# cambridge-mlg/RECOMBINER

Measured on AMD Instinct MI355X. Metric: INRs trained/sec (whole node) + PSNR@bpp vs reference, CIFAR-10, higher is better.
Workload: dtype bf16; 1 GPU; CIFAR-10 32x32, 4096 INRs/GPU, 3x32 SIREN (in 32 = 16 Fourier + 16 upsampled pe), S=1, training_mappings=True, Adam lr 2e-4; inrs_per_gpu=4096, parallelism=datapoint-sharded x1, tuned_library_gemms=True

## Files before the change

### recombiner_amd/csrc/upconv.hip

```cpp
#include "rcb_common.h"

using namespace rcb;

typedef float f32x16 __attribute__((ext_vector_type(16)));
typedef __bf16 bf16x8 __attribute__((ext_vector_type(8)));
typedef __bf16 bf16x4 __attribute__((ext_vector_type(4)));
typedef short s16x4 __attribute__((ext_vector_type(4)));

namespace {

constexpr int CIN = 64;
#ifndef RCB_UP_HOT
#define RCB_UP_HOT 0
#endif
#ifndef RCB_UP_NOSTORE
#define RCB_UP_NOSTORE 0
#endif
#ifndef RCB_B3_PF
#define RCB_B3_PF 2
#endif
#ifndef RCB_UP_PF
#define RCB_UP_PF 3
#endif
constexpr int XRS = 72;
// ... 588 lines not shown
  }
  if (b < a.batch) {
    RCB_STAGED2(img)
    if (b + gs < a.batch) RCB_FETCHD2(b + gs)
  }
  __syncthreads();
  int cur = 0;
  for (; b < a.batch; b += gs, cur ^= 1) {
    const __bf16* im = img + cur * (IMGB / 2);
    D2_T(0);
    if (b + gs < a.batch) {
      __bf16* nx = img + (cur ^ 1) * (IMGB / 2);
      RCB_STAGED2(nx)
      if (b + 2 * gs < a.batch) RCB_FETCHD2(b + 2 * gs)
    }
    D2_T(1);
    const long long xoff = ((long long)b * G * G + pos) * CIN + 32 * mt + 16 * h;
    float xf[16];
    Frag xb[2];
    if (kh == 0) {
      if (X_F32) {
#pragma unroll
        for (int k = 0; k < 4; ++k) {
          const float4 t = reinterpret_cast<const float4*>(reinterpret_cast<const float*>(a.x) + xoff)[k];
          xf[4 * k] = t.x; xf[4 * k + 1] = t.y; xf[4 * k + 2] = t.z; xf[4 * k + 3] = t.w;
        }
      } else {
        xb[0].u = reinterpret_cast<const uint4*>(reinterpret_cast<const __bf16*>(a.x) + xoff)[0];
        xb[1].u = reinterpret_cast<const uint4*>(reinterpret_cast<const __bf16*>(a.x) + xoff)[1];
      }
    }
    f32x16 acc;
#pragma unroll
    for (int r = 0; r < 16; ++r) acc[r] = 0.f;
#pragma unroll
    for (int c = 0; c < 8; ++c) {
      const int n = 8 * kh + c, ry = (n >> 2) - 1, rx = (n & 3) - 1;
      const int xx = 2 * v + rx + 1, sw = (xx >> 1) & 7;
      const __bf16* px = im + (2 * u + ry + 1) * ROWS + xx * RS;
      uint4 curf[4];
#pragma unroll
      for (int kb = 0; kb < 4; ++kb) curf[kb] = *reinterpret_cast<const uint4*>(px + 8 * ((2 * kb + h) ^ sw));
#pragma unroll
      for (int kb = 0; kb < 4; ++kb) {
        Frag bf, fa;
        bf.u = curf[kb];
        fa.u = fr[c][kb];
        acc = mfma16(fa.v, bf.v, acc);
      }
      __builtin_amdgcn_sched_barrier(0);
    }
    D2_T(3);
    float* rw = red + (cur * 4 + (wave & 3)) * 16 * 64;
    if (kh == 1) {
#pragma unroll
      for (int r = 0; r < 16; ++r) rw[r * 64 + lane] = acc[r];
    }
    D2_T(4);
    __syncthreads();
    D2_T(5);
    if (kh == 0) {
#pragma unroll
      for (int r = 0; r < 16; ++r) acc[r] += rw[r * 64 + lane];
#pragma unroll
      for (int hf = 0; hf < 2; ++hf) {
        float o[8];
#pragma unroll
        for (int k = 0; k < 4; ++k) {
          auto sw = __builtin_amdgcn_permlane32_swap(__float_as_uint(acc[4 * hf + k]), __float_as_uint(acc[8 + 4 * hf + k]),
                                                     false, false);
          o[k] = __uint_as_float(sw[0]);
          o[4 + k] = __uint_as_float(sw[1]);
        }
        if (X_F32) {
#pragma unroll
          for (int k = 0; k < 8; ++k) {
            o[k] *= (xf[8 * hf + k] > 0.f ? 1.0f : SLOPE);
            dbsum[8 * hf + k] += o[k];
          }
          float4* dst = reinterpret_cast<float4*>(reinterpret_cast<float*>(a.dx) + xoff + 8 * hf);
          dst[0] = make_float4(o[0], o[1], o[2], o[3]);
          dst[1] = make_float4(o[4], o[5], o[6], o[7]);
        } else {
          Frag oo;
#pragma unroll
          for (int k = 0; k < 8; ++k) {
            oo.v[k] = (__bf16)(o[k] * ((float)xb[hf].v[k] > 0.f ? 1.0f : SLOPE));
            dbsum[8 * hf + k] += (float)oo.v[k];
          }
          if (RCB_UP_NOSTORE != 2 || a.batch < 0) reinterpret_cast<uint4*>(reinterpret_cast<__bf16*>(a.dx) + xoff)[hf] = oo.u;
        }
      }
    }
    D2_T(6);
  }
#if RCB_D2_STAMPS
  ph_[7] = __builtin_amdgcn_s_memrealtime() - t_loop_;
  ph_[2] = t_loop_ - t_entry_;
  if (blockIdx.x == 0 && lane == 0)
    for (int k = 0; k < 8; ++k) g_d2_stamps[wave * 8 + k] = ph_[k];
#endif
#undef RCB_FETCHD2
#undef RCB_STAGED2
  if (dbias_partial) {
    __syncthreads();
#pragma unroll
    for (int k = 0; k < 16; ++k) {
#pragma unroll
      for (int off = 16; off > 0; off >>= 1) dbsum[k] += __shfl_xor(dbsum[k], off, 64);
    }
    float* r2 = red;
    if (kh == 0 && q == 0) {
#pragma unroll
      for (int k = 0; k < 16; ++k) r2[tile * 64 + 32 * mt + 16 * h + k] = dbsum[k];
    }
    __syncthreads();
    if (tid < 64) dbias_partial[(long long)blockIdx.x * 64 + tid] = r2[tid] + r2[64 + tid];
  }
}

struct WgradArgs {
  const void* x;
  const void* dy;
  float* partial;
  int batch;
};

__device__ __forceinline__ s16x4 tr_read(const __bf16* p) {
  return __builtin_amdgcn_ds_read_tr16_b64_v4i16((__attribute__((address_space(3))) s16x4*)p);
}

template <int COUT>
__device__ __forceinline__ void bias_partials_join(const float (&dbsum)[8], float* red, int tid, float* dst) {
  constexpr int C8 = COUT / 8, NG = 512 / COUT;
  __syncthreads();
#pragma unroll
  for (int j = 0; j < 8; ++j) red[tid * 8 + j] = dbsum[j];
  __syncthreads();
  {
    const int ch = tid % COUT, grp = tid / COUT;
    const int c8 = ch >> 3, j = ch & 7;
    float sacc = 0.f;
#pragma unroll
    for (int k = 0; k < 8; ++k) sacc += red[(c8 + C8 * (8 * grp + k)) * 8 + j];
    red[512 * 8 + grp * COUT + ch] = sacc;
  }
  __syncthreads();
  if (tid < COUT) {
    float tot = 0.f;
#pragma unroll
    for (int g = 0; g < NG; ++g) tot += red[512 * 8 + g * COUT + tid];
    dst[tid] = tot;
  }
}

template <int COUT, int G, int X_MODE, int DY_F32>
__global__ void __launch_bounds__(512) upconv_wgrad_kernel(WgradArgs a) {
  constexpr int NT = (COUT + 31) / 32;
  WC_T(0, 0);
  constexpr int HG = G + 2;
  constexpr int OG = 2 * G;
  constexpr int DM = DY_F32 ? 2 : 0;
  constexpr int NX = G * G * (CIN / 8) / 512, ND = OG * OG * (COUT / 8) / 512;
  static_assert(NX * 512 == G * G * (CIN / 8) && ND * 512 == OG * OG * (COUT / 8) && 512 % (COUT / 8) == 0, "tiling");
  constexpr int WSZ = 1024 * COUT, ROW = WSZ + COUT;
  extern __shared__ __attribute__((aligned(16))) unsigned char smem_raw[];
  __bf16* ximg = reinterpret_cast<__bf16*>(smem_raw);
  constexpr int DRS = COUT == 64 ? XRS : COUT;
  __bf16* dimg = ximg + HG * HG * XRS;
  const int tid = threadIdx.x, wave = tid >> 6, lane = tid & 63;
  const int h = lane >> 5, fb = (lane >> 4) & 1, i16 = lane & 15, q4 = i16 >> 2, p4 = i16 & 3;
  for (int e = tid; e < HG * HG * XRS / 8; e += 512) reinterpret_cast<uint4*>(ximg)[e] = make_uint4(0, 0, 0, 0);
  f32x16 acc[2][2][NT];
#pragma unroll
  for (int c = 0; c < 2; ++c)
#pragma unroll
    for (int mt = 0; mt < 2; ++mt)
#pragma unroll
      for (int nt = 0; nt < NT; ++nt)
#pragma unroll
        for (int r = 0; r < 16; ++r) acc[c][mt][nt][r] = 0.f;
  float dbsum[8];
#pragma unroll
  for (int j = 0; j < 8; ++j) dbsum[j] = 0.f;
  Raw8<X_MODE> px[NX];
  Raw8<DM> pd[ND];
#define RCB_WG_FETCH(bb)                                                                                   \
  {                                                                                                        \
    _Pragma("unroll") for (int k = 0; k < NX; ++k)                                                         \
        px[k] = raw_load<X_MODE>(a.x, (long long)(bb) * G * G * CIN + 8 * (tid + 512 * k));                \
    _Pragma("unroll") for (int k = 0; k < ND; ++k)                                                         \
        pd[k] = raw_load<DM>(a.dy, (long long)(bb) * OG * OG * COUT + 8 * (tid + 512 * k));                \
  }
  int b = blockIdx.x;
  if (b < a.batch) RCB_WG_FETCH(b)
  WC_T(0, 1);
  for (; b < a.batch; b += gridDim.x) {
    __syncthreads();
#pragma unroll
    for (int k = 0; k < NX; ++k) {
      const int e = tid + 512 * k, pix = e >> 3, c8 = e & 7;
      const int i = pix / G, j = pix - i * G;
      Frag f;
      f.v = raw_frag<X_MODE>(px[k], true);
      *reinterpret_cast<uint4*>(ximg + ((i + 1) * HG + (j + 1)) * XRS + 8 * c8) = f.u;
    }
#pragma unroll
    for (int k = 0; k < ND; ++k) {
      Frag f;
      f.v = raw_frag<DM>(pd[k], true);
      const int e = tid + 512 * k;
      *reinterpret_cast<uint4*>(dimg + (e / (COUT / 8)) * DRS + 8 * (e % (COUT / 8))) = f.u;
#pragma unroll
      for (int j = 0; j < 8; ++j) dbsum[j] += (float)f.v[j];
    }
    __syncthreads();
    if (b + (int)gridDim.x < a.batch) RCB_WG_FETCH(b + gridDim.x)
    {
      const int p = wave >> 1, pa = p >> 1, pb = p & 1, ty = wave & 1;
      for (int pt = 0; pt < G * G / 32; ++pt) {
#pragma unroll
        for (int ks = 0; ks < 2; ++ks) {
          union { s16x4 s[2]; bf16x8 v; } av[2][2], bv[NT];
#pragma unroll
          for (int w2 = 0; w2 < 2; ++w2) {
            const int pos = 32 * pt + 16 * ks + 8 * h + 4 * w2 + q4;
            const int i = pos / G, j = pos - i * G;
            const __bf16* xr = ximg + ((i + pa + ty) * HG + (j + pb)) * XRS + 16 * fb + 4 * p4;
#pragma unroll
            for (int c = 0; c < 2; ++c)
#pragma unroll
              for (int mt = 0; mt < 2; ++mt) av[c][mt].s[w2] = tr_read(xr + c * XRS + 32 * mt);
            const __bf16* dr = dimg + ((2 * i + pa) * OG + (2 * j + pb)) * DRS + 4 * p4;
#pragma unroll
            for (int nt = 0; nt < NT; ++nt) bv[nt].s[w2] = tr_read(dr + ((COUT >= 32) ? (32 * nt + 16 * fb) : 0));
          }
#pragma unroll
          for (int c = 0; c < 2; ++c)
#pragma unroll
            for (int mt = 0; mt < 2; ++mt)
#pragma unroll
              for (int nt = 0; nt < NT; ++nt) acc[c][mt][nt] = mfma16(av[c][mt].v, bv[nt].v, acc[c][mt][nt]);
        }
      }
    }
  }
#undef RCB_WG_FETCH
  WC_T(0, 2);
  float* slab = a.partial + (long long)blockIdx.x * ROW;
  bias_partials_join<COUT>(dbsum, reinterpret_cast<float*>(smem_raw), tid, slab + WSZ);
#pragma unroll
  for (int c = 0; c < 2; ++c) {
    const int combo = 2 * wave + c;
    const int p = combo >> 2, t = combo & 3;
#pragma unroll
    for (int mt = 0; mt < 2; ++mt)
#pragma unroll
      for (int nt = 0; nt < NT; ++nt) {
        const int co = 32 * nt + (lane & 31);
        if (co < COUT) {
#pragma unroll
          for (int r = 0; r < 16; ++r) {
            const int ci = 32 * mt + rho(r, h);
            slab[weff_index(t >> 1, t & 1, ci, p >> 1, p & 1, co, COUT)] = acc[c][mt][nt][r];
          }
        }
      }
  }
  WC_T(0, 3);
}

#ifndef RCB_B3_STAMPS
#define RCB_B3_STAMPS 0
#endif
#ifndef RCB_B3_WG16
#define RCB_B3_WG16 1
#endif
#ifndef RCB_B3_DIAG
#define RCB_B3_DIAG 0
#endif
#if RCB_B3_STAMPS
__device__ unsigned long long g_b3_stamps[8 * 8];
#define B3_T(k)                                                     \
  do {                                                              \
    const unsigned long long now_ = __builtin_amdgcn_s_memtime();   \
    ph_[k] += now_ - last_;                                         \
    last_ = now_;                                                   \
  } while (0)
#else
#define B3_T(k) do { } while (0)
#endif

struct Bwd3Args {
  const void* dy;
  const float* weff;
  const void* x;
  void* dx;
  float* partial;
  int batch;
  const uint4* pack;
};

__global__ void __launch_bounds__(512) upconv_bwd3_fused_kernel(Bwd3Args a) {
  constexpr int COUT = 16, G = 16, OG = 32, HO = 34, RS = 24, HG = 18, NF = 32;
#if RCB_B3_STAMPS
  const unsigned long long t_entry_ = __builtin_amdgcn_s_memrealtime();
#endif
  constexpr int WSZ = 1024 * COUT, ROW = WSZ + COUT;
#if RCB_B3_WG16
  constexpr int XR3 = 64;
#define B3_XKEY(col) ((((col) >> 1) & 1) | ((((col) >> 3) & 1) << 1))
#else
  constexpr int XR3 = XRS;
#define B3_XKEY(col) 0
#endif
  extern __shared__ __attribute__((aligned(16))) unsigned char smem_raw[];
  uint4* frags = reinterpret_cast<uint4*>(smem_raw);
  __bf16* dyimg = reinterpret_cast<__bf16*>(smem_raw + NF * 1024);
  __bf16* ximg = dyimg + HO * HO * RS;
  constexpr int SCR_RS = 40;
  __bf16* dxscr = ximg + HG * HG * XR3;
  const int tid = threadIdx.x, wave = tid >> 6, lane = tid & 63, q = lane & 31, h = lane >> 5;
  const int fb = (lane >> 4) & 1, i16 = lane & 15, q4 = i16 >> 2, p4 = i16 & 3;
  if (a.pack) {
    uint4 t4[NF * 64 / 512];
#pragma unroll
    for (int k = 0; k < NF * 64 / 512; ++k) t4[k] = a.pack[20480 + tid + 512 * k];
#pragma unroll
    for (int k = 0; k < NF * 64 / 512; ++k) frags[tid + 512 * k] = t4[k];
  }
  for (int e = tid; e < (a.pack ? 0 : NF * 64); e += 512) {
    const int ln = e & 63, slot = e >> 6;
    const int mt = slot & 1, combo = slot >> 1;
    const int ry = (combo >> 2) - 1, rx = (combo & 3) - 1;
    const int pa = (ry & 1), ty = (ry <= 0) ? 1 : 0;
    const int pb = (rx & 1), tx = (rx <= 0) ? 1 : 0;
    const int fq = ln & 31, fh = ln >> 5, ci = 32 * mt + fq;
    Frag f;
#pragma unroll
    for (int j = 0; j < 8; ++j) f.v[j] = (__bf16)a.weff[weff_index(ty, tx, ci, pa, pb, 8 * fh + j, COUT)];
    frags[e] = f.u;
  }
  for (int e = tid; e < (HO * HO * RS + HG * HG * XR3) / 8; e += 512) reinterpret_cast<uint4*>(dyimg)[e] = make_uint4(0, 0, 0, 0);
#if RCB_B3_WG16
  f32x4v wacc[2][4];
#pragma unroll
  for (int c = 0; c < 2; ++c)
#pragma unroll
    for (int cb = 0; cb < 4; ++cb)
#pragma unroll
      for (int r = 0; r < 4; ++r) wacc[c][cb][r] = 0.f;
#else
  f32x16 wacc[2][2];
#pragma unroll
  for (int c = 0; c < 2; ++c)
#pragma unroll
    for (int mt = 0; mt < 2; ++mt)
#pragma unroll
      for (int r = 0; r < 16; ++r) wacc[c][mt][r] = 0.f;
#endif
  float dbsum[8];
#pragma unroll
  for (int j = 0; j < 8; ++j) dbsum[j] = 0.f;
  uint4 pdy[4], px[4];
#pragma unroll
  for (int k = 0; k < 4; ++k) pdy[k] = px[k] = make_uint4(0, 0, 0, 0);
#define RCB_FETCH_B3(bb)                                                                                               \
  {                                                                                                                   \
    const uint4* sd_ = reinterpret_cast<const uint4*>(reinterpret_cast<const __bf16*>(a.dy) + (long long)(bb) * OG * OG * COUT); \
    const uint4* sx_ = reinterpret_cast<const uint4*>(reinterpret_cast<const __bf16*>(a.x) + (long long)(bb) * G * G * CIN);    \
    _Pragma("unroll") for (int k = 0; k < 4; ++k) { pdy[k] = sd_[tid + 512 * k]; px[k] = sx_[tid + 512 * k]; }         \
  }
  const int gs = gridDim.x;
  int b = blockIdx.x;
  __syncthreads();
  if (b < a.batch) RCB_FETCH_B3(b)
  const int u = (wave * 32 + q) >> 4, v = (wave * 32 + q) & 15;
#if RCB_B3_STAMPS
  unsigned long long ph_[8] = {0, 0, 0, 0, 0, 0, 0, 0}, last_ = __builtin_amdgcn_s_memtime();
  ph_[5] = __builtin_amdgcn_s_memrealtime();
#endif
  for (; b < a.batch; b += gs) {
    __syncthreads();
    B3_T(0);
#pragma unroll
    for (int k = 0; k < 4; ++k) {
      const int e = tid + 512 * k;
      {
        const int pix = e >> 1, c8 = e & 1;
        *reinterpret_cast<uint4*>(dyimg + (((pix >> 5) + 1) * HO + ((pix & 31) + 1)) * RS + 8 * c8) = pdy[k];
        Frag f;
        f.u = pdy[k];
#pragma unroll
        for (int j = 0; j < 8; ++j) dbsum[j] += (float)f.v[j];
      }
      {
        const int pix = e >> 3, c8 = e & 7;
        *reinterpret_cast<uint4*>(ximg + (((pix >> 4) + 1) * HG + ((pix & 15) + 1)) * XR3 + 16 * ((c8 >> 1) ^ B3_XKEY((pix & 15) + 1)) + 8 * (c8 & 1)) = px[k];
      }
    }
    B3_T(1);
    __syncthreads();
    B3_T(2);
    if (b + gs < a.batch) RCB_FETCH_B3(b + gs)
    {
      f32x16 acc[2];
#pragma unroll
      for (int mt = 0; mt < 2; ++mt)
#pragma unroll
        for (int r = 0; r < 16; ++r) acc[mt][r] = 0.f;
      constexpr int B3_PF = RCB_B3_PF;
      uint4 rg[B3_PF + 1][3];
      auto tap_reads = [&](int n, uint4 (&dst)[3]) {
        const int ry = (n >> 2) - 1, rx = (n & 3) - 1;
        dst[0] = *reinterpret_cast<const uint4*>(dyimg + ((2 * u + ((RCB_B3_DIAG == 3) ? 0 : ry) + 1) * HO + (2 * v + ((RCB_B3_DIAG == 3) ? 0 : rx) + 1)) * RS + 8 * h);
        dst[1] = frags[((RCB_B3_DIAG == 2 ? 0 : n) * 2 + 0) * 64 + lane];
        dst[2] = frags[((RCB_B3_DIAG == 2 ? 0 : n) * 2 + 1) * 64 + lane];
      };
#pragma unroll
      for (int n = 0; n < B3_PF; ++n) tap_reads(n, rg[n]);
#pragma unroll
      for (int n = 0; n < 16; ++n) {
        if (n + B3_PF < 16) tap_reads(n + B3_PF, rg[(n + B3_PF) % (B3_PF + 1)]);
        __builtin_amdgcn_sched_barrier(0);
        Frag bf, fa;
        bf.u = rg[n % (B3_PF + 1)][0];
#pragma unroll
        for (int mt = 0; mt < 2; ++mt) {
          fa.u = rg[n % (B3_PF + 1)][1 + mt];
          acc[mt] = mfma16(fa.v, bf.v, acc[mt]);
        }
        __builtin_amdgcn_sched_barrier(0);
      }
      const __bf16* xs = ximg + ((u + 1) * HG + (v + 1)) * XR3;
      const int xk16 = 16 * B3_XKEY(v + 1);
      __bf16* scr = dxscr + wave * (32 * SCR_RS);
      __bf16* dxw = reinterpret_cast<__bf16*>(a.dx) + ((long long)(RCB_B3_DIAG == 4 ? (int)blockIdx.x : b) * G * G + wave * 32) * CIN;
#pragma unroll
      for (int mt = 0; mt < 2; ++mt) {
#pragma unroll
        for (int g4 = 0; g4 < 4; ++g4) {
          const int ci = 32 * mt + 8 * g4 + 4 * h;
          const bf16x4 t = *reinterpret_cast<const bf16x4*>(xs + (((32 * mt + 8 * g4) & ~15) ^ xk16) + ((8 * g4) & 15) + 4 * h);
          bf16x4 ob;
#pragma unroll
          for (int k = 0; k < 4; ++k) ob[k] = (__bf16)(acc[mt][4 * g4 + k] * ((float)t[k] > 0.f ? 1.0f : SLOPE));
          *reinterpret_cast<bf16x4*>(scr + q * SCR_RS + 8 * g4 + 4 * h) = ob;
        }
        __builtin_amdgcn_fence(__ATOMIC_ACQ_REL, "wavefront");
#pragma unroll
        for (int ps = 0; ps < 2; ++ps) {
          const int pl = 16 * ps + (lane >> 2), ch = lane & 3;
          const uint4 o = *reinterpret_cast<const uint4*>(scr + pl * SCR_RS + 8 * ch);
          if (RCB_B3_DIAG != 1 || a.batch < 0) *reinterpret_cast<uint4*>(dxw + pl * CIN + 32 * mt + 8 * ch) = o;
        }
        __builtin_amdgcn_fence(__ATOMIC_ACQ_REL, "wavefront");
      }
    }
    __builtin_amdgcn_sched_barrier(0);
    B3_T(3);
#if RCB_B3_WG16
    {
      const int p = wave >> 1, pa = p >> 1, pb = p & 1, ty = wave & 1, kg = lane >> 4;
      typedef __attribute__((address_space(3))) s16x4* lds_tr_t;
      unsigned xa[2][2][4], da[2];
#pragma unroll
      for (int w2 = 0; w2 < 2; ++w2) {
        const int pos = 8 * kg + 4 * w2 + q4;
        const int i = pos >> 4, j = pos & 15;
#pragma unroll
        for (int c = 0; c < 2; ++c) {
          const int col = j + pb + c;
#pragma unroll
          for (int cb = 0; cb < 4; ++cb) {
            xa[w2][c][cb] = (unsigned)(size_t)(lds_tr_t)(ximg + ((i + pa + ty) * HG + col) * XR3 + 16 * (cb ^ B3_XKEY(col)) + 4 * p4);
            asm volatile("" : "+v"(xa[w2][c][cb]));
          }
        }
        da[w2] = (unsigned)(size_t)(lds_tr_t)(dyimg + ((2 * i + pa + 1) * HO + (2 * j + pb + 1)) * RS + 4 * p4);
        asm volatile("" : "+v"(da[w2]));
      }
      constexpr unsigned XSTEP = 2 * HG * XR3 * 2, DSTEP = 4 * HO * RS * 2;
#pragma unroll 1
      for (int trip = 0; trip < G * G / 64; ++trip) {
#pragma unroll
        for (int u2 = 0; u2 < 2; ++u2) {
          union { s16x4 s[2]; bf16x8 v; } av[2][4], bv;
#pragma unroll
          for (int w2 = 0; w2 < 2; ++w2) {
#pragma unroll
            for (int c = 0; c < 2; ++c)
#pragma unroll
              for (int cb = 0; cb < 4; ++cb)
                av[c][cb].s[w2] = __builtin_amdgcn_ds_read_tr16_b64_v4i16((lds_tr_t)(size_t)(xa[w2][c][cb] + (2 * trip + u2) * XSTEP));
            bv.s[w2] = __builtin_amdgcn_ds_read_tr16_b64_v4i16((lds_tr_t)(size_t)(da[w2] + (2 * trip + u2) * DSTEP));
          }
#pragma unroll
          for (int c = 0; c < 2; ++c)
#pragma unroll
            for (int cb = 0; cb < 4; ++cb) wacc[c][cb] = mfma16x32(av[c][cb].v, bv.v, wacc[c][cb]);
        }
      }
    }
#else
    {
      const int p = wave >> 1, pa = p >> 1, pb = p & 1, ty = wave & 1;
#pragma unroll 2
      for (int pt = 0; pt < G * G / 32; ++pt) {
#pragma unroll
        for (int ks = 0; ks < 2; ++ks) {
          union { s16x4 s[2]; bf16x8 v; } av[2][2], bv;
#pragma unroll
          for (int w2 = 0; w2 < 2; ++w2) {
            const int pos = 32 * pt + 16 * ks + 8 * h + 4 * w2 + q4;
            const int i = pos >> 4, j = pos & 15;
            const __bf16* xr = ximg + ((i + pa + ty) * HG + (j + pb)) * XRS + 16 * fb + 4 * p4;
#pragma unroll
            for (int c = 0; c < 2; ++c)
#pragma unroll
              for (int mt = 0; mt < 2; ++mt) av[c][mt].s[w2] = tr_read(xr + c * XRS + 32 * mt);
            bv.s[w2] = tr_read(dyimg + ((2 * i + pa + 1) * HO + (2 * j + pb + 1)) * RS + 4 * p4);
          }
#pragma unroll
          for (int c = 0; c < 2; ++c)
#pragma unroll
            for (int mt = 0; mt < 2; ++mt) wacc[c][mt] = mfma16(av[c][mt].v, bv.v, wacc[c][mt]);
        }
      }
    }
#endif
    B3_T(4);
  }
#if RCB_B3_STAMPS
  ph_[6] = __builtin_amdgcn_s_memrealtime();
  ph_[7] = t_entry_;
  if (blockIdx.x == 0 && lane == 0)
    for (int k = 0; k < 8; ++k) g_b3_stamps[wave * 8 + k] = ph_[k];
#endif
#undef RCB_FETCH_B3
#undef B3_XKEY
  float* slab = a.partial + (long long)blockIdx.x * ROW;
  bias_partials_join<COUT>(dbsum, reinterpret_cast<float*>(smem_raw), tid, slab + WSZ);
#pragma unroll
  for (int c = 0; c < 2; ++c) {
    const int combo = 2 * wave + c;
    const int p = combo >> 2, t = combo & 3;
#if RCB_B3_WG16
#pragma unroll
    for (int cb = 0; cb < 4; ++cb)
#pragma unroll
      for (int r = 0; r < 4; ++r)
        slab[weff_index(t >> 1, t & 1, 16 * cb + 4 * (lane >> 4) + r, p >> 1, p & 1, lane & 15, COUT)] = wacc[c][cb][r];
#else
#pragma unroll
    for (int mt = 0; mt < 2; ++mt) {
      const int co = lane & 31;
      if (co < COUT) {
#pragma unroll
        for (int r = 0; r < 16; ++r) {
          const int ci = 32 * mt + rho(r, h);
          slab[weff_index(t >> 1, t & 1, ci, p >> 1, p & 1, co, COUT)] = wacc[c][mt][r];
        }
      }
    }
#endif
  }
#if RCB_B3_STAMPS
  if (blockIdx.x == 0 && lane == 0) g_b3_stamps[wave * 8 + 4 + 60 - 60] = g_b3_stamps[wave * 8 + 4];
  if (blockIdx.x == 0 && lane == 0 && wave == 0) g_b3_stamps[63] = __builtin_amdgcn_s_memrealtime();
#endif
}

#if RCB_B3_STAMPS
}
#if RCB_D2_STAMPS
extern "C" int rcb_debug_d2_stamps(unsigned long long* dst, int n) {
  return (int)hipMemcpyFromSymbol(dst, HIP_SYMBOL(g_d2_stamps), sizeof(unsigned long long) * n);
}
#endif
#if RCB_WC_STAMPS
extern "C" int rcb_debug_wc_stamps(unsigned long long* dst, int n) {
  return (int)hipMemcpyFromSymbol(dst, HIP_SYMBOL(g_wc_stamps), sizeof(unsigned long long) * n);
}
#endif
#if RCB_F2_STAMPS
extern "C" int rcb_debug_f2_stamps(unsigned long long* dst, int n) {
  return (int)hipMemcpyFromSymbol(dst, HIP_SYMBOL(g_f2_stamps), sizeof(unsigned long long) * n);
}
#endif
extern "C" int rcb_debug_b3_stamps(unsigned long long* dst, int n) {
  return (int)hipMemcpyFromSymbol(dst, HIP_SYMBOL(g_b3_stamps), sizeof(unsigned long long) * n);
}
namespace {
#endif

__global__ void __launch_bounds__(256) upconv_wgrad_reduce_kernel(const float* __restrict__ partial, int nblk, int row,
                                                                  int wsz, float* __restrict__ dweff,
                                                                  float* __restrict__ dbias) {
  __shared__ float part[16][64];
  const int lane = threadIdx.x & 63, wave = threadIdx.x >> 6;
  const int j = blockIdx.x * 64 + lane;
  float s[4][8];
#pragma unroll
  for (int v = 0; v < 4; ++v)
#pragma unroll
    for (int u = 0; u < 8; ++u) s[v][u] = 0.f;
  if (j < row) {
    const float* p = partial + j;
    int w = 4 * wave;
    for (; w + 3 + 7 * 16 < nblk; w += 8 * 16) {
#pragma unroll
      for (int v = 0; v < 4; ++v)
#pragma unroll
        for (int u = 0; u < 8; ++u) s[v][u] += p[(long long)(w + v + 16 * u) * row];
    }
#pragma unroll
    for (int v = 0; v < 4; ++v) {
      int wv = w + v;
      for (; wv + 7 * 16 < nblk; wv += 8 * 16) {
#pragma unroll
        for (int u = 0; u < 8; ++u) s[v][u] += p[(long long)(wv + 16 * u) * row];
      }
      for (; wv < nblk; wv += 16) s[v][0] += p[(long long)wv * row];
    }
  }
#pragma unroll
  for (int v = 0; v < 4; ++v)
    part[4 * wave + v][lane] = ((s[v][0] + s[v][1]) + (s[v][2] + s[v][3])) + ((s[v][4] + s[v][5]) + (s[v][6] + s[v][7]));
  __syncthreads();
  if (wave == 0 && j < row) {
    float t[8];
#pragma unroll
    for (int k = 0; k < 8; ++k) t[k] = part[2 * k][lane] + part[2 * k + 1][lane];
    const float tot = ((t[0] + t[1]) + (t[2] + t[3])) + ((t[4] + t[5]) + (t[6] + t[7]));
    if (j < wsz) dweff[j] = tot;
    else if (dbias) dbias[j - wsz] = tot;
  }
}

template <typename K, typename A>
int launch(K kfn, const A& args, int grid, size_t smem, hipStream_t st, bool& ,
           int threads = 512) {
  hipError_t e = hipFuncSetAttribute(reinterpret_cast<const void*>(kfn), hipFuncAttributeMaxDynamicSharedMemorySize, 160 * 1024);
  if (e != hipSuccess) return fail((int)e, "upconv: hipFuncSetAttribute: %s", hipGetErrorString(e));
  kfn<<<grid, threads, smem, st>>>(args);
  RCB_LAUNCH_CHECK();
  return RCB_OK;
}

static bool half_wg(int batch) {
  static const bool on = [] { const char* e = getenv("RCB_UPCONV_HALF_WG"); return e && e[0] == '1'; }();
  return on && batch >= 768;
}


}

extern "C" int rcb_upconv_fwd(const void* x, int32_t x_is_f32_preact, const float* weff, const float* bias, void* y,
                              int32_t y_is_f32_linear, int32_t batch, int32_t grid, int32_t cout, const void* frag_pack,
                              rcb_stream_t stream) {
  RCB_REQUIRE(x && weff && bias && y, RCB_ERR_ARG, "upconv_fwd: null pointer");
  RCB_REQUIRE(batch > 0, RCB_ERR_SHAPE, "upconv_fwd: empty batch");
  RCB_REQUIRE((reinterpret_cast<uintptr_t>(frag_pack) & 15) == 0, RCB_ERR_ARG, "upconv_fwd: frag_pack must be 16-byte aligned");
  FwdArgs a{x, weff, bias, y, batch, reinterpret_cast<const uint4*>(frag_pack)};
  hipStream_t st = (hipStream_t)stream;
  constexpr int kFwd2Smem = 4 * 10 * 10 * 72 * 2 + 64 * 4;
  const int npair = (batch + 3) / 4;
  if (grid == 8 && cout == 64 && x_is_f32_preact == 1 && !y_is_f32_linear) {
    static bool done = false;
    return launch(upconv_fwd2_reg_kernel<1>, a, npair < 256 ? npair : 256, kFwd2Smem, st, done);
  }
  if (grid == 16 && cout == 16 && !x_is_f32_preact && y_is_f32_linear == 1) {
    static bool done = false;
    if (half_wg(batch)) return launch(upconv_fwd3_lds_kernel<16, 0, 4>, a, 768, 18 * 18 * 64 * 2, st, done, 256);
    return launch(upconv_fwd3_lds_kernel<16, 0, 8>, a, batch < 256 ? batch : 256, 18 * 18 * 64 * 2, st, done);
  }
  if (grid == 16 && cout == 16 && !x_is_f32_preact && y_is_f32_linear == 2) {
    static bool done = false;
    if (half_wg(batch)) return launch(upconv_fwd3_lds_kernel<16, 1, 4>, a, 768, 18 * 18 * 64 * 2, st, done, 256);
    return launch(upconv_fwd3_lds_kernel<16, 1, 8>, a, batch < 256 ? batch : 256, 18 * 18 * 64 * 2, st, done);
  }
  if (grid == 8 && cout == 64 && x_is_f32_preact == 2 && !y_is_f32_linear) {
    static bool done = false;
    return launch(upconv_fwd2_reg_kernel<3>, a, npair < 256 ? npair : 256, kFwd2Smem, st, done);
  }
  return fail(RCB_ERR_UNSUPPORTED, "upconv_fwd: grid=%d cout=%d in_mode=%d out_f32=%d not instantiated", grid, cout,
              x_is_f32_preact, y_is_f32_linear);
}

static inline int dgrad_blocks(int batch) { return batch < 256 ? batch : 256; }

extern "C" int32_t rcb_upconv_dgrad_partial_rows(int32_t batch) { return batch > 0 ? dgrad_blocks(batch) : 0; }

template <int X_F32>
static int launch_dgrad2(const DgradArgs& a, float* dbias_partial, hipStream_t st) {
  constexpr int kSmem = 2 * (((18 * (18 * 64 + 32) * 2 + 15) / 16) * 16) + 2 * 4 * 16 * 64 * 4;
  auto kfn = upconv_dgrad2_reg_kernel<X_F32>;
  hipError_t e = hipFuncSetAttribute(reinterpret_cast<const void*>(kfn), hipFuncAttributeMaxDynamicSharedMemorySize, 160 * 1024);
  if (e != hipSuccess) return fail((int)e, "upconv: hipFuncSetAttribute: %s", hipGetErrorString(e));
  kfn<<<dgrad_blocks(a.batch), 512, kSmem, st>>>(a, dbias_partial);
  RCB_LAUNCH_CHECK();
  return RCB_OK;
}

extern "C" int rcb_upconv_dgrad(const void* dy, int32_t dy_is_f32, const float* weff, const void* x,
                                int32_t x_is_f32_preact, void* dx, float* dbias_partial, int32_t batch, int32_t grid,
                                int32_t cout, const void* frag_pack, rcb_stream_t stream) {
  RCB_REQUIRE(dy && weff && x && dx, RCB_ERR_ARG, "upconv_dgrad: null pointer");
  RCB_REQUIRE(batch > 0, RCB_ERR_SHAPE, "upconv_dgrad: empty batch");
  RCB_REQUIRE((reinterpret_cast<uintptr_t>(frag_pack) & 15) == 0, RCB_ERR_ARG, "upconv_dgrad: frag_pack must be 16-byte aligned");
  DgradArgs a{dy, weff, x, dx, batch, reinterpret_cast<const uint4*>(frag_pack)};
  hipStream_t st = (hipStream_t)stream;
  if (grid == 8 && cout == 64 && !dy_is_f32 && x_is_f32_preact == 1) return launch_dgrad2<1>(a, dbias_partial, st);
  if (grid == 8 && cout == 64 && !dy_is_f32 && x_is_f32_preact == 2) return launch_dgrad2<0>(a, dbias_partial, st);
  RCB_REQUIRE(dbias_partial == nullptr, RCB_ERR_UNSUPPORTED, "upconv_dgrad: channel sums of dx only for the stage-2 kernels");
  if (grid == 16 && cout == 16 && dy_is_f32 && !x_is_f32_preact) {
    static bool done = false;
    return launch(upconv_dgrad3_lds_kernel<16, 0>, a, batch < 256 ? batch : 256, 32 * 1024 + 34 * 34 * 24 * 2, st, done);
  }
  if (grid == 16 && cout == 16 && !dy_is_f32 && !x_is_f32_preact) {
    static bool done = false;
    return launch(upconv_dgrad3_lds_kernel<16, 1>, a, batch < 256 ? batch : 256, 32 * 1024 + 34 * 34 * 24 * 2, st, done);
  }
  return fail(RCB_ERR_UNSUPPORTED, "upconv_dgrad: grid=%d cout=%d not instantiated", grid, cout);
}

static inline int wgrad_blocks(int batch) { return batch < 256 ? batch : 256; }

extern "C" int64_t rcb_upconv_wgrad_workspace(int32_t batch, int32_t cout) {
  if (batch <= 0 || cout <= 0) return 0;
  return (int64_t)wgrad_blocks(batch) * (1024LL * cout + cout);
}

extern "C" int rcb_upconv_wgrad(const void* x, int32_t x_is_f32_preact, const void* dy, int32_t dy_is_f32, float* dweff,
                                float* dbias, int32_t batch, int32_t grid, int32_t cout, float* workspace,
                                int64_t workspace_floats, rcb_stream_t stream) {
  RCB_REQUIRE(x && dy && dweff && workspace, RCB_ERR_ARG, "upconv_wgrad: null pointer");
  RCB_REQUIRE(batch > 0, RCB_ERR_SHAPE, "upconv_wgrad: empty batch");
  RCB_REQUIRE(workspace_floats >= rcb_upconv_wgrad_workspace(batch, cout), RCB_ERR_SHAPE,
              "upconv_wgrad: workspace of %lld floats, %lld needed", (long long)workspace_floats,
              (long long)rcb_upconv_wgrad_workspace(batch, cout));
  WgradArgs a{x, dy, workspace, batch};
  hipStream_t st = (hipStream_t)stream;
  const int g = wgrad_blocks(batch);
  int rc = RCB_ERR_UNSUPPORTED;
  bool hit = false;
#define RCB_WGRAD_CASE(cond, COUTv, Gv, XM, DF, SMEM)                                        \
  if (!hit && (cond)) {                                                                      \
    static bool done = false;                                                                \
    hit = true;                                                                              \
    rc = launch(upconv_wgrad_kernel<COUTv, Gv, XM, DF>, a, g, SMEM, st, done);               \
  }
  RCB_WGRAD_CASE(grid == 16 && cout == 16 && !x_is_f32_preact && dy_is_f32, 16, 16, 0, 1, (18 * 18 * XRS + 32 * 32 * 16) * 2)
  RCB_WGRAD_CASE(grid == 16 && cout == 16 && !x_is_f32_preact && !dy_is_f32, 16, 16, 0, 0, (18 * 18 * XRS + 32 * 32 * 16) * 2)
  RCB_WGRAD_CASE(grid == 8 && cout == 64 && x_is_f32_preact == 1 && !dy_is_f32, 64, 8, 1, 0, (10 * 10 * XRS + 16 * 16 * XRS) * 2)
  RCB_WGRAD_CASE(grid == 8 && cout == 64 && x_is_f32_preact == 2 && !dy_is_f32, 64, 8, 3, 0, (10 * 10 * XRS + 16 * 16 * XRS) * 2)
#undef RCB_WGRAD_CASE
  if (!hit) return fail(RCB_ERR_UNSUPPORTED, "upconv_wgrad: grid=%d cout=%d not instantiated", grid, cout);
  if (rc) return rc;
  const int row = 1024 * cout + cout;
  upconv_wgrad_reduce_kernel<<<(row + 63) / 64, 256, 0, st>>>(workspace, g, row, 1024 * cout, dweff, dbias);
  RCB_LAUNCH_CHECK();
  return RCB_OK;
}

extern "C" int rcb_upconv_bwd_fused(const void* dy, const float* weff, const void* x, void* dx, float* dweff, float* dbias,
                                    int32_t batch, int32_t grid, int32_t cout, float* workspace, int64_t workspace_floats,
                                    const void* frag_pack, rcb_stream_t stream) {
  RCB_REQUIRE(dy && weff && x && dx && dweff && workspace, RCB_ERR_ARG, "upconv_bwd_fused: null pointer");
  RCB_REQUIRE(batch > 0, RCB_ERR_SHAPE, "upconv_bwd_fused: empty batch");
  RCB_REQUIRE(grid == 16 && cout == 16, RCB_ERR_UNSUPPORTED, "upconv_bwd_fused: grid=%d cout=%d not instantiated", grid, cout);
  RCB_REQUIRE(workspace_floats >= rcb_upconv_wgrad_workspace(batch, cout), RCB_ERR_SHAPE,
              "upconv_bwd_fused: workspace of %lld floats, %lld needed", (long long)workspace_floats,
              (long long)rcb_upconv_wgrad_workspace(batch, cout));
  RCB_REQUIRE((reinterpret_cast<uintptr_t>(frag_pack) & 15) == 0, RCB_ERR_ARG, "upconv_bwd_fused: frag_pack must be 16-byte aligned");
  Bwd3Args a{dy, weff, x, dx, workspace, batch, reinterpret_cast<const uint4*>(frag_pack)};
  hipStream_t st = (hipStream_t)stream;
  const int g = wgrad_blocks(batch);
  static bool done = false;
  int rc = launch(upconv_bwd3_fused_kernel, a, g, 32 * 1024 + (34 * 34 * 24 + 18 * 18 * (RCB_B3_WG16 ? 64 : XRS)) * 2 + 8 * 32 * 40 * 2, st, done);
  if (rc) return rc;
  const int row = 1024 * cout + cout;
  upconv_wgrad_reduce_kernel<<<(row + 63) / 64, 256, 0, st>>>(workspace, g, row, 1024 * cout, dweff, dbias);
  RCB_LAUNCH_CHECK();
  return RCB_OK;
}
```

Baseline: 72.53 INRs trained/s.

## Keep upconv bwd weight fragments in registers and remap waves to spatial tiles

The fused upconv backward kernel now holds the 16 weight fragments per wave in VGPRs instead of shared memory, and remaps each wave to one output-channel half across two spatial tiles, so the data-grad loop reads only dy from LDS. It also adds a row-parity swizzle to the dy image to cut bank conflicts, spreads the next-batch global prefetch across the tap loop, prefetches the LeakyReLU mask early, and software-pipelines the weight-grad transposed reads. This removes 32KB of LDS and per-tap fragment LDS reads, at the cost of higher register pressure, which could lower occupancy or cause spills.

```diff
diff --git a/recombiner_amd/csrc/upconv.hip b/recombiner_amd/csrc/upconv.hip
--- a/recombiner_amd/csrc/upconv.hip
+++ b/recombiner_amd/csrc/upconv.hip
@@ -914,7 +914,7 @@
 };
 
 __global__ void __launch_bounds__(512) upconv_bwd3_fused_kernel(Bwd3Args a) {
-  constexpr int COUT = 16, G = 16, OG = 32, HO = 34, RS = 24, HG = 18, NF = 32;
+  constexpr int COUT = 16, G = 16, OG = 32, HO = 34, RS = 24, HG = 18;
 #if RCB_B3_STAMPS
   const unsigned long long t_entry_ = __builtin_amdgcn_s_memrealtime();
 #endif
@@ -927,32 +927,32 @@
 #define B3_XKEY(col) 0
 #endif
   extern __shared__ __attribute__((aligned(16))) unsigned char smem_raw[];
-  uint4* frags = reinterpret_cast<uint4*>(smem_raw);
-  __bf16* dyimg = reinterpret_cast<__bf16*>(smem_raw + NF * 1024);
+  __bf16* dyimg = reinterpret_cast<__bf16*>(smem_raw);
+#define B3_DKEY(row) (8 * (((row) >> 1) & 1))
   __bf16* ximg = dyimg + HO * HO * RS;
   constexpr int SCR_RS = 40;
   __bf16* dxscr = ximg + HG * HG * XR3;
   const int tid = threadIdx.x, wave = tid >> 6, lane = tid & 63, q = lane & 31, h = lane >> 5;
   const int fb = (lane >> 4) & 1, i16 = lane & 15, q4 = i16 >> 2, p4 = i16 & 3;
+  const int dmt = wave & 1;
+  uint4 fr[16];
   if (a.pack) {
-    uint4 t4[NF * 64 / 512];
-#pragma unroll
-    for (int k = 0; k < NF * 64 / 512; ++k) t4[k] = a.pack[20480 + tid + 512 * k];
-#pragma unroll
-    for (int k = 0; k < NF * 64 / 512; ++k) frags[tid + 512 * k] = t4[k];
-  }
-  for (int e = tid; e < (a.pack ? 0 : NF * 64); e += 512) {
-    const int ln = e & 63, slot = e >> 6;
-    const int mt = slot & 1, combo = slot >> 1;
-    const int ry = (combo >> 2) - 1, rx = (combo & 3) - 1;
-    const int pa = (ry & 1), ty = (ry <= 0) ? 1 : 0;
-    const int pb = (rx & 1), tx = (rx <= 0) ? 1 : 0;
-    const int fq = ln & 31, fh = ln >> 5, ci = 32 * mt + fq;
-    Frag f;
-#pragma unroll
-    for (int j = 0; j < 8; ++j) f.v[j] = (__bf16)a.weff[weff_index(ty, tx, ci, pa, pb, 8 * fh + j, COUT)];
-    frags[e] = f.u;
-  }
+#pragma unroll
+    for (int n = 0; n < 16; ++n) fr[n] = a.pack[20480 + (n * 2 + dmt) * 64 + lane];
+  } else {
+#pragma unroll
+    for (int n = 0; n < 16; ++n) {
+      const int ry = (n >> 2) - 1, rx = (n & 3) - 1;
+      const int pa = (ry & 1), ty = (ry <= 0) ? 1 : 0;
+      const int pb = (rx & 1), tx = (rx <= 0) ? 1 : 0;
+      Frag f;
+#pragma unroll
+      for (int j = 0; j < 8; ++j) f.v[j] = (__bf16)a.weff[weff_index(ty, tx, 32 * dmt + q, pa, pb, 8 * h + j, COUT)];
+      fr[n] = f.u;
+    }
+  }
+#pragma unroll
+  for (int n = 0; n < 16; ++n) pin(fr[n]);
   for (int e = tid; e < (HO * HO * RS + HG * HG * XR3) / 8; e += 512) reinterpret_cast<uint4*>(dyimg)[e] = make_uint4(0, 0, 0, 0);
 #if RCB_B3_WG16
   f32x4v wacc[2][4];
@@ -977,17 +977,31 @@
   uint4 pdy[4], px[4];
 #pragma unroll
   for (int k = 0; k < 4; ++k) pdy[k] = px[k] = make_uint4(0, 0, 0, 0);
-#define RCB_FETCH_B3(bb)                                                                                               \
+#define RCB_FETCH_B3(bb, k)                                                                                            \
   {                                                                                                                   \
-    const uint4* sd_ = reinterpret_cast<const uint4*>(reinterpret_cast<const __bf16*>(a.dy) + (long long)(bb) * OG * OG * COUT); \
-    const uint4* sx_ = reinterpret_cast<const uint4*>(reinterpret_cast<const __bf16*>(a.x) + (long long)(bb) * G * G * CIN);    \
-    _Pragma("unroll") for (int k = 0; k < 4; ++k) { pdy[k] = sd_[tid + 512 * k]; px[k] = sx_[tid + 512 * k]; }         \
+    const long long fb_ = RCB_B3_DIAG == 5 ? (long long)blockIdx.x : (long long)(bb);                                  \
+    const uint4* sd_ = reinterpret_cast<const uint4*>(reinterpret_cast<const __bf16*>(a.dy) + fb_ * OG * OG * COUT);    \
+    const uint4* sx_ = reinterpret_cast<const uint4*>(reinterpret_cast<const __bf16*>(a.x) + fb_ * G * G * CIN);        \
+    pdy[k] = sd_[tid + 512 * (k)];                                                                                    \
+    px[k] = sx_[tid + 512 * (k)];                                                                                     \
   }
   const int gs = gridDim.x;
   int b = blockIdx.x;
   __syncthreads();
-  if (b < a.batch) RCB_FETCH_B3(b)
-  const int u = (wave * 32 + q) >> 4, v = (wave * 32 + q) & 15;
+  if (b < a.batch) {
+#pragma unroll
+    for (int k = 0; k < 4; ++k) RCB_FETCH_B3(b, k)
+  }
+  const int u = ((wave >> 1) * 64 + q) >> 4, v = q & 15;
+  typedef unsigned u32x4 __attribute__((ext_vector_type(4)));
+  typedef __attribute__((address_space(3))) const u32x4* lds_u4_t;
+  unsigned ga[2];
+#pragma unroll
+  for (int par = 0; par < 2; ++par) {
+    ga[par] = (unsigned)(size_t)(lds_u4_t)(dyimg + (2 * u * HO + 2 * v) * RS + 8 * h + B3_DKEY(2 * u + 2 * par));
+    asm volatile("" : "+v"(ga[par]));
+  }
+  constexpr unsigned TILE_STEP = 4 * HO * RS * 2;
 #if RCB_B3_STAMPS
   unsigned long long ph_[8] = {0, 0, 0, 0, 0, 0, 0, 0}, last_ = __builtin_amdgcn_s_memtime();
   ph_[5] = __builtin_amdgcn_s_memrealtime();
@@ -1000,7 +1014,7 @@
       const int e = tid + 512 * k;
       {
         const int pix = e >> 1, c8 = e & 1;
-        *reinterpret_cast<uint4*>(dyimg + (((pix >> 5) + 1) * HO + ((pix & 31) + 1)) * RS + 8 * c8) = pdy[k];
+        *reinterpret_cast<uint4*>(dyimg + (((pix >> 5) + 1) * HO + ((pix & 31) + 1)) * RS + 8 * c8 + B3_DKEY((pix >> 5) + 1)) = pdy[k];
         Frag f;
         f.u = pdy[k];
 #pragma unroll
@@ -1014,49 +1028,55 @@
     B3_T(1);
     __syncthreads();
     B3_T(2);
-    if (b + gs < a.batch) RCB_FETCH_B3(b + gs)
+    const bool more = b + gs < a.batch;
     {
       f32x16 acc[2];
 #pragma unroll
-      for (int mt = 0; mt < 2; ++mt)
-#pragma unroll
-        for (int r = 0; r < 16; ++r) acc[mt][r] = 0.f;
+      for (int tl = 0; tl < 2; ++tl)
+#pragma unroll
+        for (int r = 0; r < 16; ++r) acc[tl][r] = 0.f;
       constexpr int B3_PF = RCB_B3_PF;
-      uint4 rg[B3_PF + 1][3];
-      auto tap_reads = [&](int n, uint4 (&dst)[3]) {
-        const int ry = (n >> 2) - 1, rx = (n & 3) - 1;
-        dst[0] = *reinterpret_cast<const uint4*>(dyimg + ((2 * u + ((RCB_B3_DIAG == 3) ? 0 : ry) + 1) * HO + (2 * v + ((RCB_B3_DIAG == 3) ? 0 : rx) + 1)) * RS + 8 * h);
-        dst[1] = frags[((RCB_B3_DIAG == 2 ? 0 : n) * 2 + 0) * 64 + lane];
-        dst[2] = frags[((RCB_B3_DIAG == 2 ? 0 : n) * 2 + 1) * 64 + lane];
+      u32x4 rg[B3_PF + 1][2];
+      auto tap_reads = [&](int n, u32x4 (&dst)[2]) {
+        const int ry = (RCB_B3_DIAG == 3) ? 0 : (n >> 2) - 1, rx = (RCB_B3_DIAG == 3) ? 0 : (n & 3) - 1;
+        const unsigned ad = ga[(ry + 1) >> 1] + ((ry + 1) * HO + (rx + 1)) * RS * 2;
+#pragma unroll
+        for (int tl = 0; tl < 2; ++tl) dst[tl] = *(lds_u4_t)(size_t)(ad + tl * TILE_STEP);
       };
 #pragma unroll
       for (int n = 0; n < B3_PF; ++n) tap_reads(n, rg[n]);
+      const int xk16 = 16 * B3_XKEY(v + 1);
+      bf16x4 sg[2][4];
 #pragma unroll
       for (int n = 0; n < 16; ++n) {
+        if (more && (n & 3) == 0) RCB_FETCH_B3(b + gs, n >> 2)
         if (n + B3_PF < 16) tap_reads(n + B3_PF, rg[(n + B3_PF) % (B3_PF + 1)]);
+        if (n >= 14) {
+#pragma unroll
+          for (int g4 = 0; g4 < 4; ++g4)
+            sg[n - 14][g4] = *reinterpret_cast<const bf16x4*>(ximg + ((u + 2 * (n - 14) + 1) * HG + (v + 1)) * XR3 + (((32 * dmt + 8 * g4) & ~15) ^ xk16) + ((8 * g4) & 15) + 4 * h);
+        }
         __builtin_amdgcn_sched_barrier(0);
-        Frag bf, fa;
-        bf.u = rg[n % (B3_PF + 1)][0];
-#pragma unroll
-        for (int mt = 0; mt < 2; ++mt) {
-          fa.u = rg[n % (B3_PF + 1)][1 + mt];
-          acc[mt] = mfma16(fa.v, bf.v, acc[mt]);
+        Frag fa;
+        union { u32x4 r; bf16x8 v; } bf;
+        fa.u = fr[RCB_B3_DIAG == 2 ? 0 : n];
+#pragma unroll
+        for (int tl = 0; tl < 2; ++tl) {
+          bf.r = rg[n % (B3_PF + 1)][tl];
+          acc[tl] = mfma16(fa.v, bf.v, acc[tl]);
         }
         __builtin_amdgcn_sched_barrier(0);
       }
-      const __bf16* xs = ximg + ((u + 1) * HG + (v + 1)) * XR3;
-      const int xk16 = 16 * B3_XKEY(v + 1);
       __bf16* scr = dxscr + wave * (32 * SCR_RS);
-      __bf16* dxw = reinterpret_cast<__bf16*>(a.dx) + ((long long)(RCB_B3_DIAG == 4 ? (int)blockIdx.x : b) * G * G + wave * 32) * CIN;
-#pragma unroll
-      for (int mt = 0; mt < 2; ++mt) {
+#pragma unroll
+      for (int tl = 0; tl < 2; ++tl) {
+        __bf16* dxw = reinterpret_cast<__bf16*>(a.dx) + ((long long)(RCB_B3_DIAG == 4 ? (int)blockIdx.x : b) * G * G + ((wave >> 1) * 2 + tl) * 32) * CIN;
 #pragma unroll
         for (int g4 = 0; g4 < 4; ++g4) {
-          const int ci = 32 * mt + 8 * g4 + 4 * h;
-          const bf16x4 t = *reinterpret_cast<const bf16x4*>(xs + (((32 * mt + 8 * g4) & ~15) ^ xk16) + ((8 * g4) & 15) + 4 * h);
+          const bf16x4 t = sg[tl][g4];
           bf16x4 ob;
 #pragma unroll
-          for (int k = 0; k < 4; ++k) ob[k] = (__bf16)(acc[mt][4 * g4 + k] * ((float)t[k] > 0.f ? 1.0f : SLOPE));
+          for (int k = 0; k < 4; ++k) ob[k] = (__bf16)(acc[tl][4 * g4 + k] * ((float)t[k] > 0.f ? 1.0f : SLOPE));
           *reinterpret_cast<bf16x4*>(scr + q * SCR_RS + 8 * g4 + 4 * h) = ob;
         }
         __builtin_amdgcn_fence(__ATOMIC_ACQ_REL, "wavefront");
@@ -1064,7 +1084,7 @@
         for (int ps = 0; ps < 2; ++ps) {
           const int pl = 16 * ps + (lane >> 2), ch = lane & 3;
           const uint4 o = *reinterpret_cast<const uint4*>(scr + pl * SCR_RS + 8 * ch);
-          if (RCB_B3_DIAG != 1 || a.batch < 0) *reinterpret_cast<uint4*>(dxw + pl * CIN + 32 * mt + 8 * ch) = o;
+          if (RCB_B3_DIAG != 1 || a.batch < 0) *reinterpret_cast<uint4*>(dxw + pl * CIN + 32 * dmt + 8 * ch) = o;
         }
         __builtin_amdgcn_fence(__ATOMIC_ACQ_REL, "wavefront");
       }
@@ -1089,29 +1109,32 @@
             asm volatile("" : "+v"(xa[w2][c][cb]));
           }
         }
-        da[w2] = (unsigned)(size_t)(lds_tr_t)(dyimg + ((2 * i + pa + 1) * HO + (2 * j + pb + 1)) * RS + 4 * p4);
+        da[w2] = (unsigned)(size_t)(lds_tr_t)(dyimg + ((2 * i + pa + 1) * HO + (2 * j + pb + 1)) * RS + 4 * p4 + B3_DKEY(2 * i + pa + 1));
         asm volatile("" : "+v"(da[w2]));
       }
       constexpr unsigned XSTEP = 2 * HG * XR3 * 2, DSTEP = 4 * HO * RS * 2;
-#pragma unroll 1
-      for (int trip = 0; trip < G * G / 64; ++trip) {
-#pragma unroll
-        for (int u2 = 0; u2 < 2; ++u2) {
-          union { s16x4 s[2]; bf16x8 v; } av[2][4], bv;
-#pragma unroll
-          for (int w2 = 0; w2 < 2; ++w2) {
-#pragma unroll
-            for (int c = 0; c < 2; ++c)
-#pragma unroll
-              for (int cb = 0; cb < 4; ++cb)
-                av[c][cb].s[w2] = __builtin_amdgcn_ds_read_tr16_b64_v4i16((lds_tr_t)(size_t)(xa[w2][c][cb] + (2 * trip + u2) * XSTEP));
-            bv.s[w2] = __builtin_amdgcn_ds_read_tr16_b64_v4i16((lds_tr_t)(size_t)(da[w2] + (2 * trip + u2) * DSTEP));
-          }
-#pragma unroll
-          for (int c = 0; c < 2; ++c)
-#pragma unroll
-            for (int cb = 0; cb < 4; ++cb) wacc[c][cb] = mfma16x32(av[c][cb].v, bv.v, wacc[c][cb]);
-        }
+      struct Tr8 { union { s16x4 s[2]; bf16x8 v; }; };
+      constexpr int NU = 2 * (G * G / 32);
+      Tr8 av[3][4], bv[2];
+      auto unit_reads = [&](int un) {
+        const int blk = un >> 1, c = un & 1;
+#pragma unroll
+        for (int w2 = 0; w2 < 2; ++w2) {
+#pragma unroll
+          for (int cb = 0; cb < 4; ++cb)
+            av[un % 3][cb].s[w2] = __builtin_amdgcn_ds_read_tr16_b64_v4i16((lds_tr_t)(size_t)(xa[w2][c][cb] + blk * XSTEP));
+          if (c == 0) bv[blk & 1].s[w2] = __builtin_amdgcn_ds_read_tr16_b64_v4i16((lds_tr_t)(size_t)(da[w2] + blk * DSTEP));
+        }
+      };
+      unit_reads(0);
+      unit_reads(1);
+#pragma unroll
+      for (int un = 0; un < NU; ++un) {
+        if (un + 2 < NU) unit_reads(un + 2);
+        __builtin_amdgcn_sched_barrier(0);
+#pragma unroll
+        for (int cb = 0; cb < 4; ++cb) wacc[un & 1][cb] = mfma16x32(av[un % 3][cb].v, bv[(un >> 1) & 1].v, wacc[un & 1][cb]);
+        __builtin_amdgcn_sched_barrier(0);
       }
     }
 #else
@@ -1131,7 +1154,7 @@
             for (int c = 0; c < 2; ++c)
 #pragma unroll
               for (int mt = 0; mt < 2; ++mt) av[c][mt].s[w2] = tr_read(xr + c * XRS + 32 * mt);
-            bv.s[w2] = tr_read(dyimg + ((2 * i + pa + 1) * HO + (2 * j + pb + 1)) * RS + 4 * p4);
+            bv.s[w2] = tr_read(dyimg + ((2 * i + pa + 1) * HO + (2 * j + pb + 1)) * RS + 4 * p4 + B3_DKEY(2 * i + pa + 1));
           }
 #pragma unroll
           for (int c = 0; c < 2; ++c)
@@ -1151,6 +1174,7 @@
 #endif
 #undef RCB_FETCH_B3
 #undef B3_XKEY
+#undef B3_DKEY
   float* slab = a.partial + (long long)blockIdx.x * ROW;
   bias_partials_join<COUT>(dbsum, reinterpret_cast<float*>(smem_raw), tid, slab + WSZ);
 #pragma unroll
@@ -1390,7 +1414,7 @@
   hipStream_t st = (hipStream_t)stream;
   const int g = wgrad_blocks(batch);
   static bool done = false;
-  int rc = launch(upconv_bwd3_fused_kernel, a, g, 32 * 1024 + (34 * 34 * 24 + 18 * 18 * (RCB_B3_WG16 ? 64 : XRS)) * 2 + 8 * 32 * 40 * 2, st, done);
+  int rc = launch(upconv_bwd3_fused_kernel, a, g, (34 * 34 * 24 + 18 * 18 * (RCB_B3_WG16 ? 64 : XRS)) * 2 + 8 * 32 * 40 * 2, st, done);
   if (rc) return rc;
   const int row = 1024 * cout + cout;
   upconv_wgrad_reduce_kernel<<<(row + 63) / 64, 256, 0, st>>>(workspace, g, row, 1024 * cout, dweff, dbias);
```

Result: no change. 72.98 INRs trained/s, median of 4 (+0.6%).
